# tartarughina/S-BLAS

Hardware: AMD Instinct MI355X
Metric: SpMM GFLOP/s (2*nnz*N/t), CSR x dense N=64, fp64 (higher is better)
Workload: dtype f64

## Files before the change

s-blas_amd/csrc/kernels.hip:

```cpp
#include <hip/hip_runtime.h>
#include <atomic>
#include <stdint.h>
#include <stdlib.h>
#include <algorithm>
#include <type_traits>
#include <string.h>
#include <stdio.h>
#include <mutex>
#include <vector>
#include "kernels.h"

namespace sblas {

constexpr int WAVE = 64;

__device__ __forceinline__ int wave_uniform(int v) { return __builtin_amdgcn_readfirstlane(v); }

__device__ __forceinline__ double readlane_f64(double v, int src_lane)
{
    int lo = __double2loint(v), hi = __double2hiint(v);
    lo = __builtin_amdgcn_readlane(lo, src_lane);
    hi = __builtin_amdgcn_readlane(hi, src_lane);
    return __hiloint2double(hi, lo);
}
// ... 360 lines not shown
            for (int m = 32; m > 0; m >>= 1) {
                nblk += __shfl_xor(nblk, m, WAVE);
                nchunk += __shfl_xor(nchunk, m, WAVE);
            }
            float need = mfma_min_fill;
            bool dense_chunks = true;
            if (window_ok && mfma_min_fill > 0.0f) need = fmaxf(need, 0.68f);
            if (!window_ok && mfma_min_fill > 0.0f) {
                dense_chunks = nblk >= 2 * nchunk;
                if (nblk >= 3 * nchunk) need *= 0.84f;
            }
            mfma = dense_chunks && __builtin_amdgcn_ballot_w64(!in_range) == 0ull &&
                   (float)(e1 - e0) >= need * (float)(r1 - r0) * 4.0f * (float)nblk;
        }
    }
    bool wave_rows = false;
    if (sane && !window_ok && (merge_probe & 2)) {
        int hl = 0, hr = 0;
        head_row(hl, hr);
        const int prow = min(panel_rows, rows - p * panel_rows);
        wave_rows = (hl > 0 && 5 * head_adj >= 2 * hl) || (float)mlen * (float)prow > 2.0f * (float)nnz + 16.0f * (float)prow;
    }
    if (lane == 0) {
        info[p] = last >= first ? make_int2(first, last) : make_int2(1, 0);
        const int c = mfma ? (window_ok ? PANEL_MFMA_W : PANEL_MFMA_D) : (window_ok ? PANEL_WINDOW : PANEL_DIRECT);
        cls[p] = c | (shared ? PANEL_SHARED_ROWS : 0) | (phase << PANEL_PHASE_SHIFT) | (wave_rows ? PANEL_WAVE_ROWS : 0);
        if (p == npanels / 2) tail[TAIL_BAND] = last >= first ? last - first + 1 : 0;
        if (c == PANEL_DIRECT) tail[TAIL_DIRECT_EPOCH] = epoch;
        if (c == PANEL_MFMA_D) tail[TAIL_MFMAD_EPOCH] = epoch;
        if (c == PANEL_MFMA_W || c == PANEL_MFMA_D) tail[TAIL_MFMA_EPOCH] = epoch;
    }
}
__global__ __launch_bounds__(256) void classify_panels_kernel(int rows, int cols, int npanels, int panel_rows,
                                                             const int *__restrict__ rowptr,
                                                             const int *__restrict__ colidx, int max_row_len,
                                                             float min_density, float min_rowlen, float mfma_min_fill, int merge_probe,
                                                             int *__restrict__ tail, int2 *__restrict__ info,
                                                             int *__restrict__ cls, int epoch)
{
    __shared__ unsigned bitmap[4][MFMA_BITMAP_WORDS];
    classify_panel(blockIdx.x * 4 + (threadIdx.x >> 6), rows, cols, npanels, panel_rows, rowptr, colidx, max_row_len,
                   min_density, min_rowlen, mfma_min_fill, merge_probe, tail, info, cls, epoch, bitmap[threadIdx.x >> 6]);
}
template <bool RB>
__global__ __launch_bounds__(256) void stage_classify_kernel(int64_t cols, int64_t n, const double *__restrict__ B,
                                                            int64_t ldb, double *__restrict__ Bt, int64_t ldbt,
                                                            int stage_blocks, int rows, int npanels, int panel_rows,
                                                            const int *__restrict__ rowptr,
                                                            const int *__restrict__ colidx, int max_row_len,
                                                            float min_density, float min_rowlen, float mfma_min_fill, int merge_probe,
                                                            int *__restrict__ tail, int2 *__restrict__ info,
                                                            int *__restrict__ cls, int epoch)
{
    static_assert(sizeof(double) * 64 * (STAGE_K + 1) >= sizeof(unsigned) * 4 * MFMA_BITMAP_WORDS, "LDS area");
    __shared__ double tile[64][STAGE_K + 1];
    const int cblocks = (npanels + 3) / 4;
    if ((int)blockIdx.x >= cblocks) {
        stage_tile<RB>(tile, (int64_t)((int)blockIdx.x - cblocks) * STAGE_K, (int64_t)blockIdx.y * 64, cols, n, B, ldb, Bt,
                       ldbt, tail, epoch);
    } else if (blockIdx.y == 0) {
        classify_panel((int)blockIdx.x * 4 + (threadIdx.x >> 6), rows, (int)cols, npanels, panel_rows, rowptr, colidx,
                       max_row_len, min_density, min_rowlen, mfma_min_fill, merge_probe, tail, info, cls, epoch,
                       reinterpret_cast<unsigned *>(&tile[0][0]) + (threadIdx.x >> 6) * MFMA_BITMAP_WORDS);
    }
}
__global__ __launch_bounds__(256) void colrange_classify_kernel(int64_t nnz, int2 *__restrict__ part, int nparts, int rows,
                                                               int cols, int npanels, int panel_rows,
                                                               const int *__restrict__ rowptr,
                                                               const int *__restrict__ colidx, int max_row_len,
                                                               float min_density, float min_rowlen, float mfma_min_fill, int merge_probe,
                                                               int *__restrict__ tail, int2 *__restrict__ info,
                                                               int *__restrict__ cls, int epoch)
{
    __shared__ unsigned bitmaps[4 * MFMA_BITMAP_WORDS];
    const int cblocks = (npanels + 3) / 4;
    if ((int)blockIdx.x >= cblocks)
        colrange_part(nnz, colidx, part, (int)blockIdx.x - cblocks, nparts, reinterpret_cast<int2 *>(bitmaps));
    else
        classify_panel((int)blockIdx.x * 4 + (threadIdx.x >> 6), rows, cols, npanels, panel_rows, rowptr, colidx,
                       max_row_len, min_density, min_rowlen, mfma_min_fill, merge_probe, tail, info, cls, epoch,
                       bitmaps + (threadIdx.x >> 6) * MFMA_BITMAP_WORDS);
}
template <int NC, bool RB>
__global__ __launch_bounds__(256) void stage_classify_narrow_kernel(int64_t cols, int64_t n, const double *__restrict__ B,
                                                                   int64_t ldb, double *__restrict__ Bt, int rows,
                                                                   int npanels, int panel_rows,
                                                                   const int *__restrict__ rowptr,
                                                                   const int *__restrict__ colidx, int max_row_len,
                                                                   float min_density, float min_rowlen, int *__restrict__ tail,
                                                                   int2 *__restrict__ info, int *__restrict__ cls,
                                                                   int epoch)
{
    const int cblocks = (npanels + 3) / 4;
    if ((int)blockIdx.x >= cblocks)
        stage_rows_narrow<NC, RB>((int64_t)((int)blockIdx.x - cblocks) * 256, cols, n, B, ldb, Bt, tail, epoch);
    else
        classify_panel((int)blockIdx.x * 4 + (threadIdx.x >> 6), rows, (int)cols, npanels, panel_rows, rowptr, colidx,
                       max_row_len, min_density, min_rowlen, 2.0f, 0, tail, info, cls, epoch, nullptr);
}
__global__ __launch_bounds__(1024) void mfma_vote_kernel(int npanels, int *__restrict__ tail, const int2 *__restrict__ info,
                                                       int *__restrict__ cls, int epoch, int mfma_forced)
{
    __shared__ int counts[4];
    if (threadIdx.x < 4) counts[threadIdx.x] = 0;
    __syncthreads();
    constexpr int VU = 8;
    int mine = 0, all = 0, beyond = 0, groups = 0;
    for (int p0 = threadIdx.x; p0 < npanels; p0 += VU * 1024) {
        int2 sp[VU];
        int w[VU];
#pragma unroll
        for (int u = 0; u < VU; ++u) {
            const int p = p0 + u * 1024;
            sp[u] = p < npanels ? info[p] : make_int2(1, 0);
            w[u] = p < npanels ? cls[p] : 0;
        }
#pragma unroll
        for (int u = 0; u < VU; ++u) {
            const int c = w[u] & PANEL_CLASS_MASK;
            if (sp[u].x <= sp[u].y) {
                ++all;
                mine += c == PANEL_MFMA_W || c == PANEL_MFMA_D;
                if (c == PANEL_DIRECT || c == PANEL_MFMA_D) {
                    ++beyond;
                    groups += (w[u] & PANEL_SHARED_ROWS) != 0;
                }
            }
        }
    }
    auto tally = [&](int slot, int v) {
#pragma unroll
        for (int m = 32; m > 0; m >>= 1) v += __shfl_xor(v, m, WAVE);
        if ((threadIdx.x & 63) == 0 && v != 0) atomicAdd(&counts[slot], v);
    };
    tally(0, mine);
    tally(1, all);
    tally(2, beyond);
    tally(3, groups);
    __syncthreads();
    const bool demote = !mfma_forced && counts[0] > 0 && 4 * counts[0] < 3 * counts[1];
    const bool to_merge = !mfma_forced && counts[2] > 0 && 2 * counts[3] >= counts[2];
    __syncthreads();
    if (threadIdx.x < 4) counts[threadIdx.x] = 0;
    __syncthreads();
    int direct = 0, shared = 0, left = 0, by_wave = 0;
    bool any_direct = false;
    for (int p0 = threadIdx.x; p0 < npanels; p0 += VU * 1024) {
        int2 sp[VU];
        int w[VU];
#pragma unroll
        for (int u = 0; u < VU; ++u) {
            const int p = p0 + u * 1024;
            sp[u] = p < npanels ? info[p] : make_int2(1, 0);
            w[u] = p < npanels ? cls[p] : PANEL_WINDOW;
        }
#pragma unroll
        for (int u = 0; u < VU; ++u) {
            const int p = p0 + u * 1024;
            int c = w[u] & PANEL_CLASS_MASK;
            const int flag = w[u] & ~PANEL_CLASS_MASK;
            if (p < npanels && (demote || (to_merge && c == PANEL_MFMA_D))) {
                if (c == PANEL_MFMA_W) c = PANEL_WINDOW;
                if (c == PANEL_MFMA_D) {
                    c = PANEL_DIRECT;
                    any_direct = true;
                }
                cls[p] = c | flag;
            }
            left += c == PANEL_MFMA_W || c == PANEL_MFMA_D;
            if (c == PANEL_DIRECT && sp[u].x <= sp[u].y) {
                ++direct;
                shared += (flag & PANEL_SHARED_ROWS) != 0;
                by_wave += (flag & PANEL_WAVE_ROWS) != 0;
            }
        }
    }
    tally(2, direct);
    tally(3, shared);
    tally(0, left);
    tally(1, by_wave);
    if (any_direct) tail[TAIL_DIRECT_EPOCH] = epoch;
    __syncthreads();
    if (threadIdx.x == 0) {
        if (counts[0] == 0) tail[TAIL_MFMA_EPOCH] = 0;
        if (counts[2] > 0 && 2 * counts[3] >= counts[2]) tail[TAIL_MERGE_EPOCH] = epoch;
        else if (counts[2] > 0 && 2 * counts[1] < counts[2]) tail[TAIL_ROWS_EPOCH] = epoch;
    }
}
__device__ __forceinline__ bool nothing_direct(const int *__restrict__ tail, int epoch)
{
    if (tail[TAIL_DIRECT_EPOCH] == epoch) return false;
    return !(tail[TAIL_MFMAD_EPOCH] == epoch && tail[TAIL_NONFINITE] == tail[TAIL_STAGE_EPOCH]);
}
__device__ __forceinline__ bool b_nonfinite(const int *__restrict__ tail)
{
    return tail[TAIL_NONFINITE] == tail[TAIL_STAGE_EPOCH];
}
__device__ __forceinline__ bool owns_direct(const int *__restrict__ tail, const int *__restrict__ cls, int p)
{
    const int c = cls[p] & PANEL_CLASS_MASK;
    return c == PANEL_DIRECT || (c == PANEL_MFMA_D && b_nonfinite(tail));
}
__device__ __forceinline__ bool owns_window(const int *__restrict__ tail, const int *__restrict__ cls, int p)
{
    const int c = cls[p] & PANEL_CLASS_MASK;
    return c == PANEL_WINDOW || (c == PANEL_MFMA_W && b_nonfinite(tail));
}
__device__ __forceinline__ bool is_split_row(const unsigned *__restrict__ bits, int r)
{
    return (bits[r >> 5] >> (r & 31)) & 1u;
}

typedef int sblas_rsrc_t __attribute__((ext_vector_type(4)));
__device__ __forceinline__ sblas_rsrc_t make_rsrc(const void *p, unsigned stride, unsigned records)
{
    const unsigned long long a = (unsigned long long)p;
    sblas_rsrc_t r;
    r.x = (int)(unsigned)a;
    r.y = (int)(((unsigned)(a >> 32) & 0xffffu) | (stride << 16));
    r.z = (int)records;
    r.w = 0x00020000;
    return r;
}

#define SBLAS_QSTEP4(K0, K1, K2, K3)                                                                                 \
    asm volatile("s_nop 1\n\t"                                                                                       \
                 "v_add_u32_dpp v92, %[co], %[lb] row_newbcast:" #K0 " row_mask:0xf bank_mask:0xf\n\t"               \
                 "v_add_u32_dpp v93, %[co], %[lb] row_newbcast:" #K1 " row_mask:0xf bank_mask:0xf\n\t"               \
                 "v_add_u32_dpp v94, %[co], %[lb] row_newbcast:" #K2 " row_mask:0xf bank_mask:0xf\n\t"               \
                 "v_add_u32_dpp v95, %[co], %[lb] row_newbcast:" #K3 " row_mask:0xf bank_mask:0xf\n\t"               \
                 "s_nop 0\n\t"                                                                                       \
                 "ds_read_b128 v[96:99], v92\n\t"                                                                    \
                 "ds_read_b128 v[100:103], v92 offset:256\n\t"                                                       \
                 "ds_read_b128 v[104:107], v93\n\t"                                                                  \
                 "ds_read_b128 v[108:111], v93 offset:256\n\t"                                                       \
                 "ds_read_b128 v[112:115], v94\n\t"                                                                  \
                 "ds_read_b128 v[116:119], v94 offset:256\n\t"                                                       \
                 "ds_read_b128 v[120:123], v95\n\t"                                                                  \
                 "ds_read_b128 v[124:127], v95 offset:256\n\t"                                                       \
                 "s_waitcnt lgkmcnt(7)\n\t"                                                                          \
                 "v_fmac_f64_dpp %[c0], %[gv], v[96:97] row_newbcast:" #K0 " row_mask:0xf bank_mask:0xf\n\t"         \
                 "v_fmac_f64_dpp %[c1], %[gv], v[98:99] row_newbcast:" #K0 " row_mask:0xf bank_mask:0xf\n\t"         \
                 "s_waitcnt lgkmcnt(6)\n\t"                                                                          \
                 "v_fmac_f64_dpp %[c2], %[gv], v[100:101] row_newbcast:" #K0 " row_mask:0xf bank_mask:0xf\n\t"       \
                 "v_fmac_f64_dpp %[c3], %[gv], v[102:103] row_newbcast:" #K0 " row_mask:0xf bank_mask:0xf\n\t"       \
                 "s_waitcnt lgkmcnt(5)\n\t"                                                                          \
                 "v_fmac_f64_dpp %[c0], %[gv], v[104:105] row_newbcast:" #K1 " row_mask:0xf bank_mask:0xf\n\t"       \
                 "v_fmac_f64_dpp %[c1], %[gv], v[106:107] row_newbcast:" #K1 " row_mask:0xf bank_mask:0xf\n\t"       \
                 "s_waitcnt lgkmcnt(4)\n\t"                                                                          \
                 "v_fmac_f64_dpp %[c2], %[gv], v[108:109] row_newbcast:" #K1 " row_mask:0xf bank_mask:0xf\n\t"       \
                 "v_fmac_f64_dpp %[c3], %[gv], v[110:111] row_newbcast:" #K1 " row_mask:0xf bank_mask:0xf\n\t"       \
                 "s_waitcnt lgkmcnt(3)\n\t"                                                                          \
                 "v_fmac_f64_dpp %[c0], %[gv], v[112:113] row_newbcast:" #K2 " row_mask:0xf bank_mask:0xf\n\t"       \
                 "v_fmac_f64_dpp %[c1], %[gv], v[114:115] row_newbcast:" #K2 " row_mask:0xf bank_mask:0xf\n\t"       \
                 "s_waitcnt lgkmcnt(2)\n\t"                                                                          \
                 "v_fmac_f64_dpp %[c2], %[gv], v[116:117] row_newbcast:" #K2 " row_mask:0xf bank_mask:0xf\n\t"       \
                 "v_fmac_f64_dpp %[c3], %[gv], v[118:119] row_newbcast:" #K2 " row_mask:0xf bank_mask:0xf\n\t"       \
                 "s_waitcnt lgkmcnt(1)\n\t"                                                                          \
                 "v_fmac_f64_dpp %[c0], %[gv], v[120:121] row_newbcast:" #K3 " row_mask:0xf bank_mask:0xf\n\t"       \
                 "v_fmac_f64_dpp %[c1], %[gv], v[122:123] row_newbcast:" #K3 " row_mask:0xf bank_mask:0xf\n\t"       \
                 "s_waitcnt lgkmcnt(0)\n\t"                                                                          \
                 "v_fmac_f64_dpp %[c2], %[gv], v[124:125] row_newbcast:" #K3 " row_mask:0xf bank_mask:0xf\n\t"       \
                 "v_fmac_f64_dpp %[c3], %[gv], v[126:127] row_newbcast:" #K3 " row_mask:0xf bank_mask:0xf\n\t"       \
                 : [c0] "+v"(q0), [c1] "+v"(q1), [c2] "+v"(q2), [c3] "+v"(q3)                                        \
                 : [co] "v"(co), [lb] "v"(lb), [gv] "v"(gv)                                                          \
                 : "memory", "v92", "v93", "v94", "v95", "v96", "v97", "v98", "v99", "v100", "v101", "v102", "v103", \
                   "v104", "v105", "v106", "v107", "v108", "v109", "v110", "v111", "v112", "v113", "v114", "v115",   \
                   "v116", "v117", "v118", "v119", "v120", "v121", "v122", "v123", "v124", "v125", "v126", "v127")

__device__ __forceinline__ void dma_rows_scalar(unsigned lds_addr, unsigned voff, const char *base)
{
    asm volatile("s_mov_b32 m0, %0\n\ts_nop 0\n\tglobal_load_lds_dwordx4 %1, %2" ::"s"(lds_addr), "v"(voff), "s"(base)
                 : "memory");
}
__device__ __forceinline__ void dma_rows_vector(unsigned lds_addr, const char *addr)
{
    asm volatile("s_mov_b32 m0, %0\n\ts_nop 0\n\tglobal_load_lds_dwordx4 %1, off" ::"s"(lds_addr), "v"(addr)
                 : "memory");
}

static_assert(4 * 4 * 2 >= SPMM_MIN_PANEL_ROWS, "the workspace reserves one verdict per SPMM_MIN_PANEL_ROWS rows");
constexpr int W6_GMAX = 3;


__device__ __forceinline__ void window_select6(int wc, double wv, int tile_lo, int rem, int k, unsigned zero_rel,
                                               unsigned &co, double &gv, unsigned long long &m)
{
    int glo, ghi;
    asm volatile("v_subrev_u32 %[co], %[tlo], %[wc]\n\t"
                 "v_cmp_gt_i32 %[m], %[rem], %[k]\n\t"
                 "v_cmp_gt_u32 vcc, %[tr], %[co]\n\t"
                 "v_lshlrev_b32 %[co], 9, %[co]\n\t"
                 "s_and_b64 vcc, vcc, %[m]\n\t"
                 "s_mov_b64 %[m], vcc\n\t"
                 "v_cndmask_b32 %[co], %[zr], %[co], vcc\n\t"
                 "v_cndmask_b32 %[glo], 0, %[vlo], vcc\n\t"
                 "v_cndmask_b32 %[ghi], 0, %[vhi], vcc"
                 : [co] "=&v"(co), [m] "=&s"(m), [glo] "=&v"(glo), [ghi] "=&v"(ghi)
                 : [tlo] "s"(tile_lo), [wc] "v"(wc), [rem] "v"(rem), [k] "v"(k), [zr] "v"(zero_rel),
                   [vlo] "v"(__double2loint(wv)), [vhi] "v"(__double2hiint(wv)), [tr] "n"(W2_ROWS)
                 : "vcc", "scc");
    gv = __hiloint2double(ghi, glo);
}
__device__ __forceinline__ void window_issue6(sblas_rsrc_t rc, sblas_rsrc_t rv, int idx, int &ca, double &va, int &cb,
                                              double &vb)
{
    const int idx2 = idx + 16;
    asm volatile("buffer_load_dword %0, %4, %6, 0 idxen\n\t"
                 "buffer_load_dwordx2 %1, %4, %7, 0 idxen\n\t"
                 "buffer_load_dword %2, %5, %6, 0 idxen\n\t"
                 "buffer_load_dwordx2 %3, %5, %7, 0 idxen"
                 : "=&v"(ca), "=&v"(va), "=&v"(cb), "=&v"(vb)
                 : "v"(idx), "v"(idx2), "s"(rc), "s"(rv)
                 : "memory");
}
template <int NEWER> __device__ __forceinline__ void window_wait6(int &ca, double &va, int &cb, double &vb)
{
    static_assert(NEWER == 0 || NEWER == 4 || NEWER == 8, "counts of the sixth-generation tile loop");
    if (NEWER == 4) asm volatile("s_waitcnt vmcnt(4)" : "+v"(ca), "+v"(va), "+v"(cb), "+v"(vb)::"memory");
    else if (NEWER == 8) asm volatile("s_waitcnt vmcnt(8)" : "+v"(ca), "+v"(va), "+v"(cb), "+v"(vb)::"memory");
    else asm volatile("s_waitcnt vmcnt(0)" : "+v"(ca), "+v"(va), "+v"(cb), "+v"(vb)::"memory");
}
template <int N> __device__ __forceinline__ void vm_wait6()
{
    static_assert(N == 8 || N == 12, "counts of the sixth-generation tile loop");
    if (N == 12) asm volatile("s_waitcnt vmcnt(12)" ::: "memory");
    else asm volatile("s_waitcnt vmcnt(8)" ::: "memory");
}

template <int G, int NH, bool RC>
__global__ __launch_bounds__(1024) void spmm_window6_kernel(
    int rows, int cols, int npanels, const int *__restrict__ rowptr, const int *__restrict__ colidx,
    const double *__restrict__ val, const double *__restrict__ Bt, int64_t ldbt, int n, double alpha, double beta,
    double *__restrict__ C, int64_t ldc, const int *__restrict__ tail, const int2 *__restrict__ info,
    const int *__restrict__ cls, int panel_rows, int nnz)
{
    constexpr int RW = 4 * G, RMAX = 16 * RW;
    static_assert(G == 2 || G == 3, "two or three groups per wave (the counted vmcnt waits are 4 G)");
    static_assert(NH == 1 || NH == 2, "one or two 64-column halves per workgroup");
    static_assert(64 * (RMAX + 1) <= 2 * W2_TILE, "C tile must fit in the (dead) B tile buffers");
    extern __shared__ __attribute__((aligned(16))) double smem[];
    double *zero_row = smem + 2 * W2_TILE;
    int *sm_i = reinterpret_cast<int *>(smem + 2 * W2_TILE + 64);

    const int panel = xcd_contiguous_panel(blockIdx.x, npanels);
    if (!owns_window(tail, cls, panel)) return;
    const int2 span = info[panel];

    const int tid = threadIdx.x;
    const int lane = tid & 63;
    const int wave = wave_uniform(tid >> 6);
    const int row0 = panel * panel_rows;
    const int col0 = blockIdx.y * (64 * NH);
    const unsigned ld32 = (unsigned)ldbt;
    const int t_lo = span.x / W2_ROWS, t_hi = span.y / W2_ROWS;
    const bool loader = wave >= 12;
    const bool active = !loader && wave * RW < panel_rows;

    if (tid < 64) zero_row[tid] = 0.0;
    if (tid == 0) sm_i[0] = 0;

    double acc[NH][G][4];
#pragma unroll
    for (int h = 0; h < NH; ++h)
#pragma unroll
        for (int g = 0; g < G; ++g)
#pragma unroll
            for (int j = 0; j < 4; ++j) acc[h][g][j] = 0.0;

    const unsigned ldb8 = ld32 * 8u;
    const unsigned piece_off = (unsigned)(col0 + ((lane & 31) << 1)) * 8u;
    const unsigned pair_off = (unsigned)(lane >> 5) * ldb8 + piece_off;
    const char *bt_bytes = reinterpret_cast<const char *>(Bt);
    int dummy = 0;
    auto dma_part = [&](int t, int h, int buf) {
        const int lw = wave - 12;
        const int r0 = t * W2_ROWS + lw * W2_LROWS;
        const unsigned lds0 = (unsigned)wave_uniform((int)((unsigned)(uintptr_t)(smem + buf * W2_TILE) + (unsigned)lw * (unsigned)(W2_LROWS * 512)));
        const unsigned hoff = (unsigned)h * 512u;
        if (r0 + W2_LROWS - 1 <= cols) {
            const char *p = bt_bytes + (size_t)((unsigned)r0 * ldb8) + hoff;
#pragma unroll
            for (int i = 0; i < W2_LROWS / 2; ++i) dma_rows_scalar(lds0 + i * 1024u, pair_off, p + (size_t)(2u * i) * ldb8);
        } else {
#pragma unroll
            for (int i = 0; i < W2_LROWS / 2; ++i) {
                const unsigned brow = (unsigned)min(r0 + 2 * i + (lane >> 5), cols);
                dma_rows_vector(lds0 + i * 1024u, bt_bytes + (size_t)(brow * ldb8 + piece_off + hoff));
            }
        }
    };

    if (loader) dma_part(t_lo, 0, 0);

    const int k = lane & 15, q = lane >> 4;
    const int wrow = min(row0 + wave * RW, rows);
    const int wstart = wave_uniform(rowptr[wrow]);
    const sblas_rsrc_t rc = make_rsrc(colidx + wstart, 4u, (unsigned)(nnz - wstart));
    const sblas_rsrc_t rv = make_rsrc(val + wstart, 8u, (unsigned)(nnz - wstart));
    int cur[G], end[G];
#pragma unroll
    for (int g = 0; g < G; ++g) {
        const int rr = wave * RW + 4 * g + q;
        const int row = row0 + rr;
        cur[g] = end[g] = 0;
        if (rr < panel_rows && row < rows) {
            cur[g] = rowptr[row] - wstart;
            end[g] = rowptr[row + 1] - wstart;
        }
    }
    unsigned long long viol = 0ull;
    int wca[G], wcb[G];
    double wva[G], wvb[G];
    unsigned s_coA[G], s_coB[G];
    double s_gvA[G], s_gvB[G];
    int s_take[G], s_mx[G];
    bool replay[G];
#pragma unroll
    for (int g = 0; g < G; ++g) {
        s_coA[g] = s_coB[g] = 0u;
        s_gvA[g] = s_gvB[g] = 0.0;
        s_take[g] = s_mx[g] = 0;
        replay[g] = false;
    }
#pragma unroll
    for (int g = 0; g < G; ++g) window_issue6(rc, rv, cur[g] + k, wca[g], wva[g], wcb[g], wvb[g]);
    asm volatile("s_waitcnt vmcnt(0)" ::: "memory");
    __syncthreads();
    int step = 0;
    for (int t = t_lo; t <= t_hi; ++t) {
        const int tile_lo = t * W2_ROWS;
        auto half = [&](auto hc) {
            constexpr int h = decltype(hc)::value;
            const int cbuf = step & 1;
            if (loader) {
                if (h + 1 < NH) dma_part(t, h + 1, cbuf ^ 1);
                else if (t < t_hi) dma_part(t + 1, 0, cbuf ^ 1);
            }
            const unsigned tile_base = (unsigned)(uintptr_t)(smem + cbuf * W2_TILE);
            const unsigned lb = tile_base + (unsigned)k * 16u;
            const unsigned zero_rel = (unsigned)(uintptr_t)zero_row - tile_base;
            auto visit = [&](auto gc) {
                constexpr int g = decltype(gc)::value;
                if (h == 0) window_wait6<NH == 1 ? 4 * (G - 1) : 4 * (G - 1 - g)>(wca[g], wva[g], wcb[g], wvb[g]);
                else if (replay[g]) window_wait6<0>(wca[g], wva[g], wcb[g], wvb[g]);
                double &q0 = acc[h][g][0], &q1 = acc[h][g][1], &q2 = acc[h][g][2], &q3 = acc[h][g][3];
                int lc = cur[g];
                bool full = h == 0 || replay[g];
                for (;;) {
                    unsigned coA, coB;
                    double gvA, gvB;
                    int take, mx;
                    if (full) {
                        const int rem = end[g] - lc;
                        unsigned long long mA, mB;
                        window_select6(wca[g], wva[g], tile_lo, rem, k, zero_rel, coA, gvA, mA);
                        window_select6(wcb[g], wvb[g], tile_lo, rem - 16, k, zero_rel, coB, gvB, mB);
                        const unsigned fa = q < 2 ? (unsigned)mA : (unsigned)(mA >> 32);
                        const unsigned fb = q < 2 ? (unsigned)mB : (unsigned)(mB >> 32);
                        const int sh = (q & 1) * 16;
                        take = __popc((fa >> sh) & 0xffffu) + __popc((fb >> sh) & 0xffffu);
                        viol |= mA ^ __builtin_amdgcn_ballot_w64(k < take);
                        viol |= mB ^ __builtin_amdgcn_ballot_w64(k + 16 < take);
                        mx = max(max(__builtin_amdgcn_readlane(take, 0), __builtin_amdgcn_readlane(take, 16)),
                                 max(__builtin_amdgcn_readlane(take, 32), __builtin_amdgcn_readlane(take, 48)));
                        if (NH > 1 && h == 0) {
                            s_coA[g] = coA, s_coB[g] = coB, s_gvA[g] = gvA, s_gvB[g] = gvB, s_take[g] = take, s_mx[g] = mx;
                        }
                    } else {
                        coA = s_coA[g], coB = s_coB[g], gvA = s_gvA[g], gvB = s_gvB[g], take = s_take[g], mx = s_mx[g];
                    }
                    asm volatile("s_setprio 1" ::: "memory");
                    {
                        const unsigned co = coA;
                        const double gv = gvA;
                        if (mx > 0) { SBLAS_QSTEP4(0, 1, 2, 3); }
                        if (mx > 4) { SBLAS_QSTEP4(4, 5, 6, 7); }
                        if (mx > 8) { SBLAS_QSTEP4(8, 9, 10, 11); }
                        if (mx > 12) { SBLAS_QSTEP4(12, 13, 14, 15); }
                    }
                    if (mx > 16) {
                        const unsigned co = coB;
                        const double gv = gvB;
                        SBLAS_QSTEP4(0, 1, 2, 3);
                        if (mx > 20) { SBLAS_QSTEP4(4, 5, 6, 7); }
                        if (mx > 24) { SBLAS_QSTEP4(8, 9, 10, 11); }
                        if (mx > 28) { SBLAS_QSTEP4(12, 13, 14, 15); }
                    }
                    asm volatile("s_setprio 0" ::: "memory");
                    lc += take;
                    const bool more = take >= 32 && lc < end[g];
                    if (__builtin_expect(__builtin_amdgcn_ballot_w64(more) == 0ull, 1)) break;
                    if (NH > 1 && h == 0) replay[g] = true;
                    window_issue6(rc, rv, lc + k, wca[g], wva[g], wcb[g], wvb[g]);
                    window_wait6<0>(wca[g], wva[g], wcb[g], wvb[g]);
                    full = true;
                }
                if (h == NH - 1) {
                    cur[g] = lc;
                    if (NH > 1) replay[g] = false;
                    window_issue6(rc, rv, cur[g] + k, wca[g], wva[g], wcb[g], wvb[g]);
                } else if (replay[g]) {
                    window_issue6(rc, rv, cur[g] + k, wca[g], wva[g], wcb[g], wvb[g]);
                }
            };
            if (active) {
                visit(std::integral_constant<int, 0>{});
                visit(std::integral_constant<int, 1>{});
                if constexpr (G > 2) visit(std::integral_constant<int, 2>{});
            }
            if (loader) asm volatile("s_waitcnt vmcnt(0)" : "+v"(dummy)::"memory");
            __syncthreads();
            ++step;
        };
        half(std::integral_constant<int, 0>{});
        if constexpr (NH > 1) half(std::integral_constant<int, 1>{});
    }
#pragma unroll
    for (int g = 0; g < G; ++g) window_wait6<0>(wca[g], wva[g], wcb[g], wvb[g]);
    int bad = viol != 0ull ? 1 : 0;
#pragma unroll
    for (int g = 0; g < G; ++g)
        if (__builtin_amdgcn_ballot_w64(cur[g] < end[g]) != 0ull) bad = 1;
    if (bad && lane == 0) atomicOr(&sm_i[0], 1);
    __syncthreads();
    const bool fell_back = sm_i[0] != 0;
    if (tid == 0 && blockIdx.y == 0) atomicAdd(&g_panel_stats[fell_back ? 2 : 0], 1ull);

    double *ctile = smem;
    const int nrows = min(panel_rows, rows - row0);
#pragma unroll
    for (int h = 0; h < NH; ++h) {
        const int colh = col0 + 64 * h;
        if (fell_back) {
            const unsigned lane_off = (unsigned)(colh + lane);
#pragma unroll
            for (int g = 0; g < G; ++g)
#pragma unroll
                for (int j = 0; j < 4; ++j) {
                    const int rr = wave * RW + 4 * g + j;
                    const int row = row0 + rr;
                    int a = 0, b = 0;
                    if (rr < panel_rows && row < rows) {
                        a = wave_uniform(rowptr[row]);
                        b = wave_uniform(rowptr[row + 1]);
                    }
                    acc[h][g][j] = row_direct(colidx, val, Bt, ld32, lane_off, lane, a, b);
                }
        }
        if (h > 0) __syncthreads();
#pragma unroll
        for (int g = 0; g < G; ++g) {
            if (fell_back) {
#pragma unroll
                for (int j = 0; j < 4; ++j) ctile[lane * (RMAX + 1) + wave * RW + 4 * g + j] = acc[h][g][j];
            } else {
                const int rr = wave * RW + 4 * g + q;
                ctile[(2 * k) * (RMAX + 1) + rr] = acc[h][g][0];
                ctile[(2 * k + 1) * (RMAX + 1) + rr] = acc[h][g][1];
                ctile[(32 + 2 * k) * (RMAX + 1) + rr] = acc[h][g][2];
                ctile[(33 + 2 * k) * (RMAX + 1) + rr] = acc[h][g][3];
            }
        }
        __syncthreads();
        const int ncols = min(64, n - colh);
        if constexpr (RC)
            store_rows_c<64>(C, ldc, row0, colh, panel_rows, nrows, ncols, 1024, alpha, beta,
                             [&](int r, int j) { return ctile[j * (RMAX + 1) + r]; }, [](int) { return true; });
        else
        for (int idx = tid; idx < 64 * panel_rows; idx += 1024) {
            const int r = idx % panel_rows, j = idx / panel_rows;
            if (r < nrows && j < ncols) {
                double *dst = C + (int64_t)(colh + j) * ldc + (row0 + r);
                const double sres = alpha * ctile[j * (RMAX + 1) + r];
                *dst = (beta == 0.0) ? sres : fma(beta, *dst, sres);
            }
        }
    }
}

constexpr int WL_TR = 256;
template <int NC, int CP> struct WlGeom {
    static constexpr int P = NC / 2;
    static constexpr unsigned ROWB = NC * 8;
    static constexpr unsigned ROW = CP * ROWB;
    static constexpr int SHIFT = ROW == 64 ? 6 : ROW == 128 ? 7 : 8;
    static constexpr unsigned TILE = WL_TR * ROW;
    static constexpr size_t LDS_BYTES = 2 * (size_t)TILE + 512 + 64;
    static constexpr int LPR = CP * P;
    static constexpr int RPI = 64 / LPR;
    static_assert(ROW == 64 || ROW == 128 || ROW == 256, "copies x row bytes");
    static_assert(CP * P <= 16, "a lane group has sixteen lanes");
};

__device__ __forceinline__ int b128_group_pos(int lane)
{
    const int l = lane & 31;
    if (l < 4) return l;
    if (l < 12) return l - 4;
    if (l < 16) return l - 8;
    if (l < 20) return l - 8;
    if (l < 28) return l - 12;
    return l - 16;
}

template <int SHIFT>
__device__ __forceinline__ void lanes_select(int wc, double wv, int tile_lo, int rem, int k, unsigned zero_rel,
                                             unsigned &co, double &gv, unsigned long long &m)
{
    int glo, ghi;
    asm volatile("v_subrev_u32 %[co], %[tlo], %[wc]\n\t"
                 "v_cmp_gt_i32 %[m], %[rem], %[k]\n\t"
                 "v_cmp_gt_u32 vcc, 0x100, %[co]\n\t"
                 "v_lshlrev_b32 %[co], %[sh], %[co]\n\t"
                 "s_and_b64 vcc, vcc, %[m]\n\t"
                 "s_mov_b64 %[m], vcc\n\t"
                 "v_cndmask_b32 %[co], %[zr], %[co], vcc\n\t"
                 "v_cndmask_b32 %[glo], 0, %[vlo], vcc\n\t"
                 "v_cndmask_b32 %[ghi], 0, %[vhi], vcc"
                 : [co] "=&v"(co), [m] "=&s"(m), [glo] "=&v"(glo), [ghi] "=&v"(ghi)
                 : [tlo] "s"(tile_lo), [wc] "v"(wc), [rem] "v"(rem), [k] "v"(k), [zr] "v"(zero_rel),
                   [vlo] "v"(__double2loint(wv)), [vhi] "v"(__double2hiint(wv)), [sh] "n"(SHIFT)
                 : "vcc", "scc");
    gv = __hiloint2double(ghi, glo);
    static_assert(WL_TR == 256, "the literal of the selection");
}
typedef double sblas_d2 __attribute__((ext_vector_type(2)));
typedef const __attribute__((address_space(3))) sblas_d2 *sblas_lds_d2;
template <int PL>
__device__ __forceinline__ void lanes_fma(unsigned lo, double gv, const unsigned long long (&wrap)[PL], sblas_d2 (&acc)[PL])
{
    constexpr int CH = PL < 4 ? PL : 4;
    const unsigned hi = lo - (unsigned)(PL * 16);
#pragma unroll
    for (int j0 = 0; j0 < PL; j0 += CH) {
        sblas_d2 b[CH];
#pragma unroll
        for (int u = 0; u < CH; ++u) {
            const int j = j0 + u;
            unsigned a = lo;
            if (j > 0) asm("v_cndmask_b32 %0, %1, %2, %3" : "=v"(a) : "v"(lo), "v"(hi), "s"(wrap[j]));
            b[u] = ((sblas_lds_d2)(uintptr_t)a)[j];
        }
#pragma unroll
        for (int u = 0; u < CH; ++u) {
            acc[j0 + u].x = fma(gv, b[u].x, acc[j0 + u].x);
            acc[j0 + u].y = fma(gv, b[u].y, acc[j0 + u].y);
        }
    }
}
__device__ __forceinline__ unsigned dpp_ror8(unsigned x) { return (unsigned)__builtin_amdgcn_update_dpp(0, (int)x, 0x128, 0xf, 0xf, false); }
__device__ __forceinline__ double dpp_ror8(double x)
{
    return __hiloint2double((int)dpp_ror8((unsigned)__double2hiint(x)), (int)dpp_ror8((unsigned)__double2loint(x)));
}
template <int NC>
__device__ __noinline__ double row_direct_narrow(const int *__restrict__ colidx, const double *__restrict__ val,
                                                 const double *__restrict__ Bt, int lane, int p0, int p1)
{
    double mine = 0.0;
    for (int j0 = 0; j0 < NC; j0 += 8) {
        double a[8];
#pragma unroll
        for (int j = 0; j < 8; ++j) a[j] = 0.0;
        for (int p = p0 + lane; p < p1; p += WAVE) {
            const double v = val[p];
            const double *br = Bt + (size_t)colidx[p] * NC + j0;
#pragma unroll
            for (int j = 0; j < 8; ++j) a[j] = fma(v, br[j], a[j]);
        }
#pragma unroll
        for (int j = 0; j < 8; ++j) {
            double s = a[j];
#pragma unroll
            for (int m = 32; m > 0; m >>= 1) s += __shfl_xor(s, m, WAVE);
            if (lane == j0 + j) mine = s;
        }
    }
    return mine;
}

template <int NC, int CP, int G, int LPE, bool RC>
__global__ __launch_bounds__(1024, (NC == 8 && CP == 1 && G == 1) ? 8 : 4) void spmm_lanes_kernel(
    int rows, int cols, int npanels, const int *__restrict__ rowptr, const int *__restrict__ colidx,
    const double *__restrict__ val, const double *__restrict__ Bt, int n, double alpha, double beta,
    double *__restrict__ C, int64_t ldc, const int *__restrict__ tail, const int2 *__restrict__ info,
    const int *__restrict__ cls, int panel_rows, int nnz)
{
    using Geo = WlGeom<NC, CP>;
    constexpr int P = Geo::P;
    constexpr int PL = P / LPE;
    constexpr unsigned WL_TILE = Geo::TILE;
    constexpr int RW = 4 * G, RMAX = 12 * RW;
    static_assert(NC == 8 || NC == 16 || NC == 32, "8, 16 or 32 dense columns");
    static_assert(LPE == 1 || (LPE == 2 && NC >= 16 && CP == 1), "two lanes per entry: 16 or 32 columns, one copy");
    static_assert(G >= 1 && G <= 3, "one to three groups of four rows per wave (counted vmcnt waits: 4 G)");
    static_assert((size_t)NC * (RMAX + 1) * sizeof(double) <= 2 * (size_t)WL_TILE, "C tile must fit in the (dead) B tiles");
    extern __shared__ __attribute__((aligned(16))) double smem[];
    char *sm = reinterpret_cast<char *>(smem);
    double *zero_row = reinterpret_cast<double *>(sm + 2 * WL_TILE);
    int *sm_i = reinterpret_cast<int *>(sm + 2 * WL_TILE + 512);

    const int panel = xcd_contiguous_panel(blockIdx.x, npanels);
    if (!owns_window(tail, cls, panel)) return;
    const int2 span = info[panel];

    const int tid = threadIdx.x;
    const int lane = tid & 63;
    const int wave = wave_uniform(tid >> 6);
    const int row0 = panel * panel_rows;
    const int t_lo = span.x / WL_TR, t_hi = span.y / WL_TR;
    const bool loader = wave >= 12;
    const bool active = !loader && wave * RW < panel_rows;

    if (tid < 64) zero_row[tid] = 0.0;
    if (tid == 0) sm_i[0] = 0;

    sblas_d2 acc[G][PL];
#pragma unroll
    for (int g = 0; g < G; ++g)
#pragma unroll
        for (int j = 0; j < PL; ++j) acc[g][j] = sblas_d2{0.0, 0.0};

    const char *bt_bytes = reinterpret_cast<const char *>(Bt);
    const unsigned dma_piece = (unsigned)((lane % Geo::LPR) & (P - 1)) * 16u;
    const unsigned dma_voff = (unsigned)(lane / Geo::LPR) * Geo::ROWB + dma_piece;
    int dummy = 0;
    auto dma_tile = [&](int t, int buf) {
        const int lw = wave - 12;
        const int r0 = t * WL_TR + lw * 64;
        const unsigned lds0 = (unsigned)(uintptr_t)(sm + (size_t)buf * WL_TILE) + (unsigned)lw * (64u * Geo::ROW);
        constexpr int NI = 64 / Geo::RPI;
        if (r0 + 63 <= cols) {
            const char *p = bt_bytes + (size_t)r0 * Geo::ROWB;
#pragma unroll
            for (int i = 0; i < NI; ++i)
                dma_rows_scalar(lds0 + i * 1024u, dma_voff, p + (size_t)(Geo::RPI * i) * Geo::ROWB);
        } else {
#pragma unroll
            for (int i = 0; i < NI; ++i) {
                const unsigned brow = (unsigned)min(r0 + Geo::RPI * i + lane / Geo::LPR, cols);
                dma_rows_vector(lds0 + i * 1024u, bt_bytes + (size_t)brow * Geo::ROWB + dma_piece);
            }
        }
    };
    if (loader) dma_tile(t_lo, 0);

    const int k = lane & 15, q = lane >> 4;
    const int gpos = b128_group_pos(lane);
    const int rot = LPE == 2 ? (k & (PL - 1)) : (gpos & (P - 1)), copy = LPE == 2 ? 0 : (gpos / P) % CP;
    const int half = LPE == 2 ? (k >> 3) : 0;
    const unsigned lane_off = (unsigned)copy * Geo::ROWB + (unsigned)half * (PL * 16u) + (unsigned)rot * 16u;
    unsigned long long wrap[PL];
#pragma unroll
    for (int j = 0; j < PL; ++j) wrap[j] = __builtin_amdgcn_ballot_w64(j + rot >= PL);
    const bool upper = k >= 8;

    const int wrow = min(row0 + wave * RW, rows);
    const int wstart = wave_uniform(rowptr[wrow]);
    const sblas_rsrc_t rc = make_rsrc(colidx + wstart, 4u, (unsigned)(nnz - wstart));
    const sblas_rsrc_t rv = make_rsrc(val + wstart, 8u, (unsigned)(nnz - wstart));
    int cur[G], end[G];
#pragma unroll
    for (int g = 0; g < G; ++g) {
        const int rr = wave * RW + 4 * g + q;
        const int row = row0 + rr;
        cur[g] = end[g] = 0;
        if (rr < panel_rows && row < rows) {
            cur[g] = rowptr[row] - wstart;
            end[g] = rowptr[row + 1] - wstart;
        }
    }
    unsigned long long viol = 0ull;
    int wca[G], wcb[G];
    double wva[G], wvb[G];
#pragma unroll
    for (int g = 0; g < G; ++g) window_issue6(rc, rv, cur[g] + k, wca[g], wva[g], wcb[g], wvb[g]);
    asm volatile("s_waitcnt vmcnt(0)" ::: "memory");
    __syncthreads();
    for (int t = t_lo; t <= t_hi; ++t) {
        const int cbuf = (t - t_lo) & 1;
        if (loader && t < t_hi) dma_tile(t + 1, cbuf ^ 1);
        const int tile_lo = t * WL_TR;
        const unsigned tile_base = (unsigned)(uintptr_t)(sm + (size_t)cbuf * WL_TILE);
        const unsigned lb = tile_base + lane_off;
        const unsigned zero_rel = (unsigned)(uintptr_t)zero_row - tile_base;
        auto visit = [&](auto gc) {
            constexpr int g = decltype(gc)::value;
            window_wait6<4 * (G - 1)>(wca[g], wva[g], wcb[g], wvb[g]);
            for (;;) {
                const int rem = end[g] - cur[g];
                unsigned coA, coB;
                double gvA, gvB;
                unsigned long long mA, mB;
                lanes_select<Geo::SHIFT>(wca[g], wva[g], tile_lo, rem, k, zero_rel, coA, gvA, mA);
                lanes_select<Geo::SHIFT>(wcb[g], wvb[g], tile_lo, rem - 16, k, zero_rel, coB, gvB, mB);
                const unsigned fa = q < 2 ? (unsigned)mA : (unsigned)(mA >> 32);
                const unsigned fb = q < 2 ? (unsigned)mB : (unsigned)(mB >> 32);
                const int sh = (q & 1) * 16;
                const int take = __popc((fa >> sh) & 0xffffu) + __popc((fb >> sh) & 0xffffu);
                viol |= mA ^ __builtin_amdgcn_ballot_w64(k < take);
                viol |= mB ^ __builtin_amdgcn_ballot_w64(k + 16 < take);
                asm volatile("s_setprio 1" ::: "memory");
                if constexpr (LPE == 1) {
                    if (mA != 0ull) lanes_fma<PL>(lb + coA, gvA, wrap, acc[g]);
                    asm volatile("" ::: "memory");
                    if (mB != 0ull) lanes_fma<PL>(lb + coB, gvB, wrap, acc[g]);
                } else {
                    const unsigned long long LOW8 = 0x00ff00ff00ff00ffull;
                    const unsigned coAr = dpp_ror8(coA), coBr = dpp_ror8(coB);
                    const double gvAr = dpp_ror8(gvA), gvBr = dpp_ror8(gvB);
                    if ((mA & LOW8) != 0ull) lanes_fma<PL>(lb + (upper ? coAr : coA), upper ? gvAr : gvA, wrap, acc[g]);
                    asm volatile("" ::: "memory");
                    if ((mA & ~LOW8) != 0ull) lanes_fma<PL>(lb + (upper ? coA : coAr), upper ? gvA : gvAr, wrap, acc[g]);
                    asm volatile("" ::: "memory");
                    if ((mB & LOW8) != 0ull) lanes_fma<PL>(lb + (upper ? coBr : coB), upper ? gvBr : gvB, wrap, acc[g]);
                    asm volatile("" ::: "memory");
                    if ((mB & ~LOW8) != 0ull) lanes_fma<PL>(lb + (upper ? coB : coBr), upper ? gvB : gvBr, wrap, acc[g]);
                }
                asm volatile("s_setprio 0" ::: "memory");
                cur[g] += take;
                const bool more = take >= 32 && cur[g] < end[g];
// ... 1547 lines not shown
```

Baseline: 15200.

## Split window prefetch into column-then-value loads and select next tile early

The window prefetch is split in two. Column indices for the next tile are loaded first and the window selection (masks, take counts, shared-memory offsets) runs right away. Value loads are then issued only for lanes that will contribute, with non-contributing lanes pointed at an out-of-range index that returns zero. This removes the saved per-group select state and the value bytes fetched for entries outside the tile, in exchange for more vmcnt bookkeeping, extra serialized waits on the replay and drain paths, and a dependent load chain.

```diff
diff --git a/s-blas_amd/csrc/kernels.hip b/s-blas_amd/csrc/kernels.hip
--- a/s-blas_amd/csrc/kernels.hip
+++ b/s-blas_amd/csrc/kernels.hip
@@ -686,6 +686,20 @@
                  : "vcc", "scc");
     gv = __hiloint2double(ghi, glo);
 }
+__device__ __forceinline__ void window_select6c(int wc, int tile_lo, int rem, int k, unsigned zero_rel, unsigned &co,
+                                                unsigned long long &m)
+{
+    asm volatile("v_subrev_u32 %[co], %[tlo], %[wc]\n\t"
+                 "v_cmp_gt_i32 %[m], %[rem], %[k]\n\t"
+                 "v_cmp_gt_u32 vcc, %[tr], %[co]\n\t"
+                 "v_lshlrev_b32 %[co], 9, %[co]\n\t"
+                 "s_and_b64 vcc, vcc, %[m]\n\t"
+                 "s_mov_b64 %[m], vcc\n\t"
+                 "v_cndmask_b32 %[co], %[zr], %[co], vcc"
+                 : [co] "=&v"(co), [m] "=&s"(m)
+                 : [tlo] "s"(tile_lo), [wc] "v"(wc), [rem] "v"(rem), [k] "v"(k), [zr] "v"(zero_rel), [tr] "n"(W2_ROWS)
+                 : "vcc", "scc");
+}
 __device__ __forceinline__ void window_issue6(sblas_rsrc_t rc, sblas_rsrc_t rv, int idx, int &ca, double &va, int &cb,
                                               double &vb)
 {
@@ -698,12 +712,38 @@
                  : "v"(idx), "v"(idx2), "s"(rc), "s"(rv)
                  : "memory");
 }
+constexpr bool w6_count(int n) { return n == 0 || n == 2 || n == 4 || n == 6 || n == 8 || n == 10; }
 template <int NEWER> __device__ __forceinline__ void window_wait6(int &ca, double &va, int &cb, double &vb)
 {
-    static_assert(NEWER == 0 || NEWER == 4 || NEWER == 8, "counts of the sixth-generation tile loop");
-    if (NEWER == 4) asm volatile("s_waitcnt vmcnt(4)" : "+v"(ca), "+v"(va), "+v"(cb), "+v"(vb)::"memory");
-    else if (NEWER == 8) asm volatile("s_waitcnt vmcnt(8)" : "+v"(ca), "+v"(va), "+v"(cb), "+v"(vb)::"memory");
-    else asm volatile("s_waitcnt vmcnt(0)" : "+v"(ca), "+v"(va), "+v"(cb), "+v"(vb)::"memory");
+    static_assert(w6_count(NEWER), "counts of the sixth-generation tile loop");
+    asm volatile("s_waitcnt vmcnt(%4)" : "+v"(ca), "+v"(va), "+v"(cb), "+v"(vb) : "n"(NEWER) : "memory");
+}
+__device__ __forceinline__ void cols_issue6(sblas_rsrc_t rc, int idx, int &ca, int &cb)
+{
+    const int idx2 = idx + 16;
+    asm volatile("buffer_load_dword %0, %2, %4, 0 idxen\n\t"
+                 "buffer_load_dword %1, %3, %4, 0 idxen"
+                 : "=&v"(ca), "=&v"(cb)
+                 : "v"(idx), "v"(idx2), "s"(rc)
+                 : "memory");
+}
+__device__ __forceinline__ void vals_issue6(sblas_rsrc_t rv, int ia, int ib, double &va, double &vb)
+{
+    asm volatile("buffer_load_dwordx2 %0, %2, %4, 0 idxen\n\t"
+                 "buffer_load_dwordx2 %1, %3, %4, 0 idxen"
+                 : "=&v"(va), "=&v"(vb)
+                 : "v"(ia), "v"(ib), "s"(rv)
+                 : "memory");
+}
+template <int NEWER> __device__ __forceinline__ void cols_wait6(int &ca, int &cb)
+{
+    static_assert(w6_count(NEWER), "counts of the sixth-generation tile loop");
+    asm volatile("s_waitcnt vmcnt(%2)" : "+v"(ca), "+v"(cb) : "n"(NEWER) : "memory");
+}
+template <int NEWER> __device__ __forceinline__ void vals_wait6(double &va, double &vb)
+{
+    static_assert(w6_count(NEWER), "counts of the sixth-generation tile loop");
+    asm volatile("s_waitcnt vmcnt(%2)" : "+v"(va), "+v"(vb) : "n"(NEWER) : "memory");
 }
 template <int N> __device__ __forceinline__ void vm_wait6()
 {
@@ -794,22 +834,47 @@
         }
     }
     unsigned long long viol = 0ull;
-    int wca[G], wcb[G];
-    double wva[G], wvb[G];
-    unsigned s_coA[G], s_coB[G];
-    double s_gvA[G], s_gvB[G];
-    int s_take[G], s_mx[G];
+    const int nrec = (int)(nnz - wstart);
+    unsigned coA[G], coB[G];
+    double gvA[G], gvB[G];
+    int take[G], mx[G], wca[G], wcb[G];
     bool replay[G];
 #pragma unroll
+    for (int g = 0; g < G; ++g) replay[g] = false;
+    auto select = [&](int g, int c, int tl, unsigned zrel, auto wv) {
+        const int rem = end[g] - c;
+        unsigned long long mA, mB;
+        if constexpr (decltype(wv)::value) {
+            window_select6(wca[g], gvA[g], tl, rem, k, zrel, coA[g], gvA[g], mA);
+            window_select6(wcb[g], gvB[g], tl, rem - 16, k, zrel, coB[g], gvB[g], mB);
+        } else {
+            window_select6c(wca[g], tl, rem, k, zrel, coA[g], mA);
+            window_select6c(wcb[g], tl, rem - 16, k, zrel, coB[g], mB);
+        }
+        const unsigned fa = q < 2 ? (unsigned)mA : (unsigned)(mA >> 32);
+        const unsigned fb = q < 2 ? (unsigned)mB : (unsigned)(mB >> 32);
+        const int sh = (q & 1) * 16;
+        const int tk = __popc((fa >> sh) & 0xffffu) + __popc((fb >> sh) & 0xffffu);
+        viol |= mA ^ __builtin_amdgcn_ballot_w64(k < tk);
+        viol |= mB ^ __builtin_amdgcn_ballot_w64(k + 16 < tk);
+        take[g] = tk;
+        mx[g] = max(max(__builtin_amdgcn_readlane(tk, 0), __builtin_amdgcn_readlane(tk, 16)),
+                    max(__builtin_amdgcn_readlane(tk, 32), __builtin_amdgcn_readlane(tk, 48)));
+    };
+    auto fetch_next = [&](int g, int c) {
+        vals_issue6(rv, k < take[g] ? c + k : nrec, k + 16 < take[g] ? c + 16 + k : nrec, gvA[g], gvB[g]);
+        cols_issue6(rc, c + take[g] + k, wca[g], wcb[g]);
+    };
+    const unsigned zero_rel0 = (unsigned)(uintptr_t)zero_row - (unsigned)(uintptr_t)smem;
+#pragma unroll
+    for (int g = 0; g < G; ++g) cols_issue6(rc, cur[g] + k, wca[g], wcb[g]);
+#pragma unroll
+    for (int g = 0; g < G; ++g) cols_wait6<0>(wca[g], wcb[g]);
+#pragma unroll
     for (int g = 0; g < G; ++g) {
-        s_coA[g] = s_coB[g] = 0u;
-        s_gvA[g] = s_gvB[g] = 0.0;
-        s_take[g] = s_mx[g] = 0;
-        replay[g] = false;
-    }
-#pragma unroll
-    for (int g = 0; g < G; ++g) window_issue6(rc, rv, cur[g] + k, wca[g], wva[g], wcb[g], wvb[g]);
-    asm volatile("s_waitcnt vmcnt(0)" ::: "memory");
+        select(g, cur[g], t_lo * W2_ROWS, zero_rel0, std::false_type{});
+        fetch_next(g, cur[g]);
+    }
     __syncthreads();
     int step = 0;
     for (int t = t_lo; t <= t_hi; ++t) {
@@ -824,68 +889,59 @@
             const unsigned tile_base = (unsigned)(uintptr_t)(smem + cbuf * W2_TILE);
             const unsigned lb = tile_base + (unsigned)k * 16u;
             const unsigned zero_rel = (unsigned)(uintptr_t)zero_row - tile_base;
+            const unsigned zero_rel_next = (unsigned)(uintptr_t)zero_row - (unsigned)(uintptr_t)(smem + (cbuf ^ 1) * W2_TILE);
             auto visit = [&](auto gc) {
                 constexpr int g = decltype(gc)::value;
-                if (h == 0) window_wait6<NH == 1 ? 4 * (G - 1) : 4 * (G - 1 - g)>(wca[g], wva[g], wcb[g], wvb[g]);
-                else if (replay[g]) window_wait6<0>(wca[g], wva[g], wcb[g], wvb[g]);
+                if (h == 0) vals_wait6<NH == 1 ? 4 * G - 2 : 2 + 4 * (G - 1 - g)>(gvA[g], gvB[g]);
                 double &q0 = acc[h][g][0], &q1 = acc[h][g][1], &q2 = acc[h][g][2], &q3 = acc[h][g][3];
                 int lc = cur[g];
-                bool full = h == 0 || replay[g];
+                bool drained = false;
+                if (h > 0 && replay[g]) {
+                    window_wait6<0>(wca[g], gvA[g], wcb[g], gvB[g]);
+                    select(g, lc, tile_lo, zero_rel, std::true_type{});
+                }
                 for (;;) {
-                    unsigned coA, coB;
-                    double gvA, gvB;
-                    int take, mx;
-                    if (full) {
-                        const int rem = end[g] - lc;
-                        unsigned long long mA, mB;
-                        window_select6(wca[g], wva[g], tile_lo, rem, k, zero_rel, coA, gvA, mA);
-                        window_select6(wcb[g], wvb[g], tile_lo, rem - 16, k, zero_rel, coB, gvB, mB);
-                        const unsigned fa = q < 2 ? (unsigned)mA : (unsigned)(mA >> 32);
-                        const unsigned fb = q < 2 ? (unsigned)mB : (unsigned)(mB >> 32);
-                        const int sh = (q & 1) * 16;
-                        take = __popc((fa >> sh) & 0xffffu) + __popc((fb >> sh) & 0xffffu);
-                        viol |= mA ^ __builtin_amdgcn_ballot_w64(k < take);
-                        viol |= mB ^ __builtin_amdgcn_ballot_w64(k + 16 < take);
-                        mx = max(max(__builtin_amdgcn_readlane(take, 0), __builtin_amdgcn_readlane(take, 16)),
-                                 max(__builtin_amdgcn_readlane(take, 32), __builtin_amdgcn_readlane(take, 48)));
-                        if (NH > 1 && h == 0) {
-                            s_coA[g] = coA, s_coB[g] = coB, s_gvA[g] = gvA, s_gvB[g] = gvB, s_take[g] = take, s_mx[g] = mx;
-                        }
-                    } else {
-                        coA = s_coA[g], coB = s_coB[g], gvA = s_gvA[g], gvB = s_gvB[g], take = s_take[g], mx = s_mx[g];
-                    }
+                    const int m = mx[g];
                     asm volatile("s_setprio 1" ::: "memory");
                     {
-                        const unsigned co = coA;
-                        const double gv = gvA;
-                        if (mx > 0) { SBLAS_QSTEP4(0, 1, 2, 3); }
-                        if (mx > 4) { SBLAS_QSTEP4(4, 5, 6, 7); }
-                        if (mx > 8) { SBLAS_QSTEP4(8, 9, 10, 11); }
-                        if (mx > 12) { SBLAS_QSTEP4(12, 13, 14, 15); }
+                        const unsigned co = coA[g];
+                        const double gv = gvA[g];
+                        if (m > 0) { SBLAS_QSTEP4(0, 1, 2, 3); }
+                        if (m > 4) { SBLAS_QSTEP4(4, 5, 6, 7); }
+                        if (m > 8) { SBLAS_QSTEP4(8, 9, 10, 11); }
+                        if (m > 12) { SBLAS_QSTEP4(12, 13, 14, 15); }
                     }
-                    if (mx > 16) {
-                        const unsigned co = coB;
-                        const double gv = gvB;
+                    if (m > 16) {
+                        const unsigned co = coB[g];
+                        const double gv = gvB[g];
                         SBLAS_QSTEP4(0, 1, 2, 3);
-                        if (mx > 20) { SBLAS_QSTEP4(4, 5, 6, 7); }
-                        if (mx > 24) { SBLAS_QSTEP4(8, 9, 10, 11); }
-                        if (mx > 28) { SBLAS_QSTEP4(12, 13, 14, 15); }
+                        if (m > 20) { SBLAS_QSTEP4(4, 5, 6, 7); }
+                        if (m > 24) { SBLAS_QSTEP4(8, 9, 10, 11); }
+                        if (m > 28) { SBLAS_QSTEP4(12, 13, 14, 15); }
                     }
                     asm volatile("s_setprio 0" ::: "memory");
-                    lc += take;
-                    const bool more = take >= 32 && lc < end[g];
+                    lc += take[g];
+                    const bool more = take[g] >= 32 && lc < end[g];
                     if (__builtin_expect(__builtin_amdgcn_ballot_w64(more) == 0ull, 1)) break;
                     if (NH > 1 && h == 0) replay[g] = true;
-                    window_issue6(rc, rv, lc + k, wca[g], wva[g], wcb[g], wvb[g]);
-                    window_wait6<0>(wca[g], wva[g], wcb[g], wvb[g]);
-                    full = true;
+                    drained = true;
+                    cols_wait6<0>(wca[g], wcb[g]);
+                    window_issue6(rc, rv, lc + k, wca[g], gvA[g], wcb[g], gvB[g]);
+                    window_wait6<0>(wca[g], gvA[g], wcb[g], gvB[g]);
+                    select(g, lc, tile_lo, zero_rel, std::true_type{});
                 }
                 if (h == NH - 1) {
                     cur[g] = lc;
+                    if (drained || (NH > 1 && replay[g])) {
+                        cols_issue6(rc, cur[g] + k, wca[g], wcb[g]);
+                        cols_wait6<0>(wca[g], wcb[g]);
+                    }
                     if (NH > 1) replay[g] = false;
-                    window_issue6(rc, rv, cur[g] + k, wca[g], wva[g], wcb[g], wvb[g]);
+                    cols_wait6<4 * (G - 1)>(wca[g], wcb[g]);
+                    select(g, cur[g], tile_lo + W2_ROWS, zero_rel_next, std::false_type{});
+                    fetch_next(g, cur[g]);
                 } else if (replay[g]) {
-                    window_issue6(rc, rv, cur[g] + k, wca[g], wva[g], wcb[g], wvb[g]);
+                    window_issue6(rc, rv, cur[g] + k, wca[g], gvA[g], wcb[g], gvB[g]);
                 }
             };
             if (active) {
@@ -901,7 +957,7 @@
         if constexpr (NH > 1) half(std::integral_constant<int, 1>{});
     }
 #pragma unroll
-    for (int g = 0; g < G; ++g) window_wait6<0>(wca[g], wva[g], wcb[g], wvb[g]);
+    for (int g = 0; g < G; ++g) window_wait6<0>(wca[g], gvA[g], wcb[g], gvB[g]);
     int bad = viol != 0ull ? 1 : 0;
 #pragma unroll
     for (int g = 0; g < G; ++g)
```

Result: no change. 15410 (median of 6 runs) (+1.4%).
